# BenjSta/bernoulli-var-speech-codec

Measured on AMD Instinct MI355X. Metric: audio-seconds coded per wall-second (encode+decode), 22.05 kHz @ 3 kbit/s, higher is better.
Workload: dtype f32; 1 GPU; BASELINE configs[1]: batch 64 x 5 s utterances per GPU, config_varBitRate @ 3000 bit/s (35 bits/frame), full encode -> BigVGAN decode; one batch at a time on one stream; frames_per_utterance=430, weights=seeded synthetic (checkpoints are LFS pointers), gather=none, streams=1

## Files before the change

### bernoulli-var-speech-codec_amd/csrc/k_vocoder.hip

```cpp
#include "k_vocoder.h"

namespace bvc {

struct ConvArgs {
    const float *in;  long long Lin;
    float *out;       long long Lout;
    long long in_bs, out_bs;
    long long row_begin;
    const float *res; const float *acc;
    const float *wp;  const float *bias;
    const float *act_a; const float *act_ib;
    float divisor;
    int epi, ks, dil, cout, ntiles, tiles_per_batch;
    const long long *row_lim;
};

template <int CIN, int NTW, int MT, bool NSPLIT = false, int SHIFT = 0>
__global__ __launch_bounds__(256) void conv_mfma_kernel(ConvArgs a) {
    extern __shared__ __attribute__((aligned(16))) float tile[];
    constexpr int S = CIN + 2;
    constexpr int TT = (NSPLIT ? 1 : 4) * MT * 16;
    constexpr int C4 = CIN / 4;
    const int tid = threadIdx.x, lane = tid & 63;
    const int wave = __builtin_amdgcn_readfirstlane(tid >> 6);
    const int r = lane & 15, g = lane >> 4;
    const int b = blockIdx.x / a.tiles_per_batch;
    const long long t0 = a.row_begin + (long long)(blockIdx.x % a.tiles_per_batch) * TT;
    const int ntile0 = NSPLIT ? (blockIdx.y * 4 + wave) * NTW : blockIdx.y * NTW;
    const int halo = (a.ks - 1) * a.dil;
    const int rows = TT + halo;
    const long long lin = a.row_lim ? a.row_lim[b] : a.Lin;

    const float *inb = a.in + (long long)b * a.in_bs;
    for (int idx = tid; idx < rows * C4; idx += 256) {
        const int row = idx / C4, c4 = idx - row * C4;
        const long long tg = t0 - halo + SHIFT + row;
        f32x4 v = (f32x4){0.f, 0.f, 0.f, 0.f};
        if (tg >= 0 && tg < lin) {
            v = *reinterpret_cast<const f32x4 *>(inb + tg * CIN + c4 * 4);
            if (a.act_a) {
                const f32x4 aa = *reinterpret_cast<const f32x4 *>(a.act_a + c4 * 4);
                const f32x4 bb = *reinterpret_cast<const f32x4 *>(a.act_ib + c4 * 4);
#pragma unroll
                for (int e = 0; e < 4; e += 2) {
                    const f32x2 o2 = snakebeta2((f32x2){v[e], v[e + 1]}, (f32x2){aa[e], aa[e + 1]}, (f32x2){bb[e], bb[e + 1]});
                    v[e] = o2[0]; v[e + 1] = o2[1];
                }
            }
        }
        park16<S>(tile, row, c4 * 4, v);
    }
    __syncthreads();

    f32x4 acc[MT][NTW];
#pragma unroll
    for (int i = 0; i < MT; ++i)
#pragma unroll
        for (int n = 0; n < NTW; ++n) acc[i][n] = (f32x4){0.f, 0.f, 0.f, 0.f};

    const int mbase = NSPLIT ? 0 : wave * MT * 16;
    const float *wl = a.wp + (long long)ntile0 * 64 + lane;
    const long long kstride = (long long)a.ntiles * 64;
    bool nok[NTW];
#pragma unroll
    for (int n = 0; n < NTW; ++n) nok[n] = (ntile0 + n) < a.ntiles;

    for (int j = 0; j < a.ks; ++j) {
        const float *arow = tile + (mbase + r + j * a.dil) * S + g;
        const float *wj = wl + (long long)j * C4 * kstride;
        constexpr int CGU = (C4 % 8 == 0) ? 8 : (C4 % 5 == 0) ? 5 : (C4 % 4 == 0) ? 4 : (C4 % 2 == 0) ? 2 : 1;
#pragma unroll 1
        for (int cg0 = 0; cg0 < C4; cg0 += CGU) {
            float bw[CGU][NTW];
#pragma unroll
            for (int u = 0; u < CGU; ++u)
#pragma unroll
                for (int n = 0; n < NTW; ++n)
                    bw[u][n] = nok[n] ? wj[(long long)(cg0 + u) * kstride + n * 64] : 0.0f;
#pragma unroll
            for (int u = 0; u < CGU; ++u) {
                float av[MT];
#pragma unroll
                for (int i = 0; i < MT; ++i) av[i] = arow[i * 16 * S + (cg0 + u) * 4];
#pragma unroll
                for (int i = 0; i < MT; ++i)
#pragma unroll
                    for (int n = 0; n < NTW; ++n)
                        acc[i][n] = __builtin_amdgcn_mfma_f32_16x16x4f32(bw[u][n], av[i], acc[i][n], 0, 0, 0);
            }
        }
    }

    const long long ob = (long long)b * a.out_bs;
#pragma unroll
    for (int i = 0; i < MT; ++i) {
        const long long t = t0 + mbase + i * 16 + r;
        if (t >= a.Lout) continue;
#pragma unroll
        for (int n = 0; n < NTW; ++n) {
            const int col = (ntile0 + n) * 16 + g * 4;
            if (col >= a.cout) continue;
            const long long o = ob + t * a.cout + col;
            f32x4 v = acc[i][n] + *reinterpret_cast<const f32x4 *>(a.bias + col);
            if (a.epi >= CE_RES) v = v + *reinterpret_cast<const f32x4 *>(a.res + o);
            if (a.epi >= CE_RES_ACC) v = *reinterpret_cast<const f32x4 *>(a.acc + o) + v;
            divide_if(a.epi == CE_RES_ACC_DIV, v, a.divisor);
            *reinterpret_cast<f32x4 *>(a.out + o) = v;
        }
    }
}

template <int CIN, int NTW, int MT, bool NSPLIT = false, int SHIFT = 0>
static int launch_one(const ConvArgs &a, int B, hipStream_t s) {
    constexpr int TT = (NSPLIT ? 1 : 4) * MT * 16;
    ConvArgs k = a;
    k.tiles_per_batch = (int)((a.Lout - a.row_begin + TT - 1) / TT);
    if (k.tiles_per_batch <= 0) return BVC_OK;
    const size_t lds = (size_t)(TT + (a.ks - 1) * a.dil) * (CIN + 2) * sizeof(float);
    if (lds > 160 * 1024) { set_error("conv tile needs %zu B of LDS", lds); return BVC_EINVAL; }
    constexpr int NPW = NTW * (NSPLIT ? 4 : 1);
    dim3 grid((unsigned)(k.tiles_per_batch * (long long)B), (unsigned)((a.ntiles + NPW - 1) / NPW));
    auto kern = conv_mfma_kernel<CIN, NTW, MT, NSPLIT, SHIFT>;
    ProbeScope probe(PK_CONV, s);
    hipLaunchKernelGGL(kern, grid, dim3(256), lds, s, k);
    BVC_HIP_TRY(hipGetLastError());
    return BVC_OK;
}

template <int CIN, int NTW, int MT, bool NSPLIT = false, int SHIFT = 0>
static int allow_big_lds() {
    BVC_HIP_TRY(hipFuncSetAttribute(reinterpret_cast<const void *>(conv_mfma_kernel<CIN, NTW, MT, NSPLIT, SHIFT>),
                                    hipFuncAttributeMaxDynamicSharedMemorySize, 160 * 1024));
    return BVC_OK;
}

__global__ void snakebeta_test_kernel(const float *__restrict__ x, long long n, float a, float ib, float *__restrict__ y) {
    for (long long i = ((long long)blockIdx.x * blockDim.x + threadIdx.x) * 2; i < n; i += (long long)gridDim.x * blockDim.x * 2) {
        if (i + 1 < n && !(i & 2)) {
            const f32x2 v = snakebeta2((f32x2){x[i], x[i + 1]}, splat2(a), splat2(ib));
            y[i] = v[0];
            y[i + 1] = v[1];
        } else {
            y[i] = snakebeta(x[i], a, ib);
            if (i + 1 < n) y[i + 1] = snakebeta(x[i + 1], a, ib);
        }
    }
}

int launch_snakebeta_test(const float *x, long long n, float a, float ib, float *y, hipStream_t s) {
    if (n <= 0) return BVC_OK;
    hipLaunchKernelGGL(snakebeta_test_kernel, dim3(256), dim3(256), 0, s, x, n, a, ib, y);
    BVC_HIP_TRY(hipGetLastError());
    return BVC_OK;
}

int conv_kernels_init() {
    int rc;
    if ((rc = amp_kernels_init())) return rc;
    if ((rc = allow_big_lds<512, 4, 1>())) return rc;
    if ((rc = allow_big_lds<512, 4, 1, true>())) return rc;
    if ((rc = allow_big_lds<256, 4, 2>())) return rc;
    if ((rc = allow_big_lds<256, 4, 1, true>())) return rc;
    if ((rc = allow_big_lds<128, 4, 2>())) return rc;
    if ((rc = allow_big_lds<80, 4, 2>())) return rc;
    if ((rc = allow_big_lds<80, 4, 2, false, 3>())) return rc;
    if ((rc = allow_big_lds<64, 4, 2>())) return rc;
    if ((rc = allow_big_lds<32, 2, 4>())) return rc;
    if ((rc = allow_big_lds<16, 1, 4>())) return rc;
    if ((rc = allow_big_lds<8, 1, 4>())) return rc;
    return BVC_OK;
}

int launch_conv_mfma(const ConvLayer &c, const float *in, long long Lin, float *out, long long Lout, int B,
                     int epi, const float *res, const float *acc, float divisor, hipStream_t s, const ConvWindow *win,
                     const long long *row_lim, long long in_bs, int shift) {
    if (B <= 0 || Lout <= 0) return BVC_OK;
    if (c.cout % 4) { set_error("conv_mfma: %d output columns (the epilogue stores 16-byte granules)", c.cout); return BVC_EINVAL; }
    ConvArgs a;
    a.in = in; a.Lin = Lin; a.out = out; a.Lout = Lout; a.res = res; a.acc = acc;
    a.in_bs = win ? win->in_bs : (in_bs ? in_bs : Lin * c.cin);
    a.out_bs = win ? win->out_bs : Lout * c.cout;
    a.row_begin = win ? win->row_begin : 0;
    a.wp = c.wp; a.bias = c.bias; a.act_a = c.act_a; a.act_ib = c.act_ib;
    a.divisor = divisor; a.epi = epi; a.ks = c.ks; a.dil = c.dil; a.cout = c.cout; a.ntiles = c.ntiles;
    a.tiles_per_batch = 0;
    a.row_lim = row_lim;
    if (shift) {
        if (shift != 3 || c.cin != 80 || c.ks != 7 || c.dil != 1 || win || row_lim) { set_error("conv_mfma: a shifted window is conv_pre's (80 channels, 7 taps, shift 3)"); return BVC_EINVAL; }
        return launch_one<80, 4, 2, false, 3>(a, B, s);
    }
    if (win && Lout - a.row_begin <= 16) {
        switch (c.cin) {
            case 512: return launch_one<512, 4, 1, true>(a, B, s);
            case 256: return launch_one<256, 4, 1, true>(a, B, s);
            case 128: return launch_one<128, 4, 1, true>(a, B, s);
            case 80:  return launch_one<80, 2, 1, true>(a, B, s);
            case 64:  return launch_one<64, 4, 1, true>(a, B, s);
            default: break;
        }
    }
    switch (c.cin) {
        case 512: return launch_one<512, 4, 1>(a, B, s);
        case 256: return launch_one<256, 4, 2>(a, B, s);
        case 128: return launch_one<128, 4, 2>(a, B, s);
        case 80:  return launch_one<80, 4, 2>(a, B, s);
        case 64:  return launch_one<64, 4, 2>(a, B, s);
        case 32:  return launch_one<32, 2, 4>(a, B, s);
        case 16:  return launch_one<16, 1, 4>(a, B, s);
        case 8:   return launch_one<8, 1, 4>(a, B, s);
        default:
            set_error("conv_mfma: unsupported input channel count %d", c.cin);
            return BVC_EINVAL;
    }
}

template <int C, int SHIFT = 0>
__global__ __launch_bounds__(256) void conv_post_kernel(const float *__restrict__ in, long long Lin, int ks,
                                                        const float *__restrict__ w, const float *__restrict__ bias,
                                                        const float *__restrict__ act_a,
                                                        const float *__restrict__ act_ib, float div,
                                                        float *__restrict__ wav, long long n_out,
                                                        int tiles_per_batch, long long in_bs, long long row_begin,
                                                        const long long *__restrict__ n_rows) {
    extern __shared__ __attribute__((aligned(16))) float tile[];
    const int tid = threadIdx.x;
    const int b = blockIdx.x / tiles_per_batch;
    const long long t0 = row_begin + (long long)(blockIdx.x % tiles_per_batch) * 256;
    const int halo = ks - 1;
    const float *inb = in + (long long)b * in_bs;
    for (int idx = tid; idx < (256 + halo) * C; idx += 256) {
        const int row = idx / C, c = idx - row * C;
        const long long tg = t0 - halo + SHIFT + row;
        float v = 0.0f;
        if (tg >= 0 && tg < Lin) v = snakebeta(inb[tg * C + c], act_a[c], act_ib[c]);
        tile[idx] = v;
    }
    __syncthreads();
    const long long t = t0 + tid - row_begin;
    if (t >= n_out) return;
    if (n_rows && t >= n_rows[b]) { wav[(long long)b * n_out + t] = 0.0f; return; }
    float acc = 0.0f;
    for (int j = 0; j < ks; ++j)
#pragma unroll
        for (int c = 0; c < C; ++c) acc = fmaf(w[c * ks + j], tile[(tid + j) * C + c], acc);
    wav[(long long)b * n_out + t] = tanhf(acc + bias[0]) / div;
}

template <int C>
__global__ __launch_bounds__(256) void conv_post_aa_kernel(const float *__restrict__ in, long long Lin, int ks,
                                                           const float *__restrict__ w, const float *__restrict__ bias,
                                                           const float *__restrict__ act_a, const float *__restrict__ act_ib,
                                                           const float *__restrict__ fu, const float *__restrict__ fd, float div,
                                                           float *__restrict__ wav, long long n_out, int tiles_per_batch) {
    extern __shared__ __attribute__((aligned(16))) float tile[];
    const int tid = threadIdx.x;
    const int b = blockIdx.x / tiles_per_batch;
    const long long t0 = (long long)(blockIdx.x % tiles_per_batch) * 256;
    const int halo = ks - 1, nact = 256 + halo, nraw = nact + 10;
    float *raw = tile + nact * C;
    const float *inb = in + (long long)b * Lin * C;
    const int first = (int)(t0 - halo) - 5;
    for (int idx = tid; idx < nraw * C; idx += 256) {
        const long long tg = first + idx / C;
        raw[idx] = (tg >= 0 && tg < Lin) ? inb[tg * C + (idx % C)] : 0.0f;
    }
    __syncthreads();
    aa_rows<C>(raw, first, nraw, Lin, tile, first + 5, nact, C, act_a, act_ib, fu, fd);
    __syncthreads();
    const long long t = t0 + tid;
    if (t >= n_out) return;
    float acc = 0.0f;
    for (int j = 0; j < ks; ++j)
#pragma unroll
        for (int c = 0; c < C; ++c) acc = fmaf(w[c * ks + j], tile[(tid + j) * C + c], acc);
    wav[(long long)b * n_out + t] = tanhf(acc + bias[0]) / div;
}

int launch_conv_post(const float *in, long long Lin, int C, int ks, const float *w, const float *bias,
                     const float *act_a, const float *act_ib, float div, float *wav, long long n_out, int B,
                     hipStream_t s, const ConvWindow *win, const long long *n_rows, const float *aa_up, const float *aa_down,
                     bool sym, long long in_bs) {
    if (B <= 0 || n_out <= 0) return BVC_OK;
    if (C != 8 && C != 16 && C != 32) { set_error("conv_post: unsupported channel count %d", C); return BVC_EINVAL; }
    const int tiles = (int)((n_out + 255) / 256);
    if (aa_up || aa_down) {
        if (sym || in_bs) { set_error("conv_post: an anti-aliased activation_post stands in front of a causal conv_post, on a dense signal"); return BVC_EINVAL; }
        if (!aa_up || !aa_down || win || n_rows) { set_error("conv_post: an anti-aliased activation_post has no streaming window and no mixed lengths"); return BVC_EINVAL; }
        if (Lin + 512 > 0x7FFFFFFFll) { set_error("conv_post: %lld rows are beyond the anti-aliased kernel's row index", Lin); return BVC_EINVAL; }
        const size_t lds_aa = (size_t)(2 * (256 + ks - 1) + 10) * C * sizeof(float);
        ProbeScope probe(PK_POST, s);
        auto kern = C == 8 ? conv_post_aa_kernel<8> : C == 16 ? conv_post_aa_kernel<16> : conv_post_aa_kernel<32>;
        if (C == 32) {
            static bool attr = false;
            if (!attr) { BVC_HIP_TRY(hipFuncSetAttribute(reinterpret_cast<const void *>(conv_post_aa_kernel<32>), hipFuncAttributeMaxDynamicSharedMemorySize, 160 * 1024)); attr = true; }
        }
        hipLaunchKernelGGL(kern, dim3((unsigned)(tiles * (long long)B)), dim3(256), lds_aa, s, in, Lin, ks,
                           w, bias, act_a, act_ib, aa_up, aa_down, div, wav, n_out, tiles);
        BVC_HIP_TRY(hipGetLastError());
        return BVC_OK;
    }
    const size_t lds = (size_t)(256 + ks - 1) * C * sizeof(float);
    if (sym && (win || n_rows || ks != 7)) { set_error("conv_post: a symmetric conv_post has 7 taps, no streaming window and no mixed lengths"); return BVC_EINVAL; }
    ProbeScope probe(PK_POST, s);
    auto kern = sym ? (C == 8 ? conv_post_kernel<8, 3> : C == 16 ? conv_post_kernel<16, 3> : conv_post_kernel<32, 3>)
                    : (C == 8 ? conv_post_kernel<8> : C == 16 ? conv_post_kernel<16> : conv_post_kernel<32>);
    hipLaunchKernelGGL(kern, dim3((unsigned)(tiles * (long long)B)), dim3(256), lds, s, in, Lin, ks,
                       w, bias, act_a, act_ib, div, wav, n_out, tiles, win ? win->in_bs : (in_bs ? in_bs : Lin * C), win ? win->row_begin : 0, n_rows);
    BVC_HIP_TRY(hipGetLastError());
    return BVC_OK;
}

struct UpRates { int u[8]; };
__global__ void ragged_limits_kernel(long long *__restrict__ lim, const long long *__restrict__ frames,
                                     const long long *__restrict__ lengths, int B, long long T, long long n_max, int n_up, UpRates r) {
    const int b = blockIdx.x * blockDim.x + threadIdx.x;
    if (b >= B) return;
    const long long f = frames[b] < 0 ? 0 : (frames[b] > T ? T : frames[b]);
    long long L = f;
    for (int i = 0; i < n_up; ++i) {
        lim[(long long)i * B + b] = L;
        L = (L + 1) * r.u[i];
    }
    long long n = lengths[b] < L ? lengths[b] : L;
    n = f == 0 ? 0 : (n < 0 ? 0 : (n > n_max ? n_max : n));
    lim[(long long)n_up * B + b] = n;
}

int launch_ragged_limits(long long *lim, const long long *frames, const long long *lengths, int B, long long T, long long n_max,
                         int n_up, const int *up_rates, hipStream_t s) {
    if (B <= 0) return BVC_OK;
    if (n_up > 8) { set_error("ragged limits: %d upsamplers", n_up); return BVC_EINVAL; }
    UpRates r;
    for (int i = 0; i < 8; ++i) r.u[i] = i < n_up ? up_rates[i] : 0;
    hipLaunchKernelGGL(ragged_limits_kernel, dim3((B + 255) / 256), dim3(256), 0, s, lim, frames, lengths, B, T, n_max, n_up, r);
    BVC_HIP_TRY(hipGetLastError());
    return BVC_OK;
}
}
```

Before: 7088 audio-seconds/s.

## Reuse staged input tile across column groups in MFMA conv and post kernel

Adds a conv_rows kernel that stages the activated input row tile in LDS once and then loops over several output column groups per block, so input loads and snake activations are no longer repeated for every column block. It also prefetches weight fragments one step ahead, swizzles block order across groups of eight, and loads input through bounds-checked buffer loads in batches of 16-byte vectors. The non-MFMA conv_post kernel gets the same vectorized buffer loading and stores its tile channel-major with padding to reduce LDS bank conflicts. The trade-offs are fewer blocks in the grid, with less parallelism for narrow layers, and more register pressure from the double-buffered weights.

After: 7100 audio-seconds/s (median of 6 runs). Within noise of the previous version (+0.2%).

```diff
diff --git a/bernoulli-var-speech-codec_amd/csrc/k_vocoder.hip b/bernoulli-var-speech-codec_amd/csrc/k_vocoder.hip
--- a/bernoulli-var-speech-codec_amd/csrc/k_vocoder.hip
+++ b/bernoulli-var-speech-codec_amd/csrc/k_vocoder.hip
@@ -13,7 +13,20 @@
     float divisor;
     int epi, ks, dil, cout, ntiles, tiles_per_batch;
     const long long *row_lim;
+    unsigned nrt;
+    int ncg;
 };
+
+struct SpanRows { __amdgpu_buffer_rsrc_t rs; int row0; };
+__device__ __forceinline__ SpanRows span_rows(const float *item, long long lin, long long first, int rows, int C) {
+    const long long in0 = first > 0 ? first : 0;
+    long long n = (first + rows < lin ? first + rows : lin) - in0;
+    if (n < 0) n = 0;
+    return {__builtin_amdgcn_make_buffer_rsrc(const_cast<float *>(item + in0 * C), 0, (int)(n * C * 4), 0x00020000), (int)(in0 - first)};
+}
+__device__ __forceinline__ f32x4 span_load4(const SpanRows &sp, int row, int C, int c0) {
+    return __builtin_bit_cast(f32x4, __builtin_amdgcn_raw_buffer_load_b128(sp.rs, ((row - sp.row0) * C + c0) * 4, 0, 0));
+}
 
 template <int CIN, int NTW, int MT, bool NSPLIT = false, int SHIFT = 0>
 __global__ __launch_bounds__(256) void conv_mfma_kernel(ConvArgs a) {
@@ -110,6 +123,166 @@
     }
 }
 
+constexpr int conv_rows_waves(int CIN) { return CIN <= 32 ? 4 : 1; }
+template <int CIN, int NTW, int MT, int SHIFT = 0>
+__global__ __launch_bounds__(256, conv_rows_waves(CIN)) void conv_rows_kernel(ConvArgs a) {
+    extern __shared__ __attribute__((aligned(16))) float tile[];
+    constexpr int S = CIN + 2;
+    constexpr int TT = 4 * MT * 16;
+    constexpr int C4 = CIN / 4;
+    constexpr int CGU = (C4 % 8 == 0) ? 8 : (C4 % 5 == 0) ? 5 : (C4 % 4 == 0) ? 4 : (C4 % 2 == 0) ? 2 : 1;
+    constexpr int CPT = C4 / CGU;
+    const int tid = threadIdx.x, lane = tid & 63;
+    const int wave = __builtin_amdgcn_readfirstlane(tid >> 6);
+    const int r = lane & 15, g = lane >> 4;
+    const unsigned per = gridDim.x >> 3;
+    const unsigned bid = (blockIdx.x & 7u) * per + (blockIdx.x >> 3);
+    if (bid >= a.nrt) return;
+    const int b = (int)(bid / (unsigned)a.tiles_per_batch);
+    const long long t0 = a.row_begin + (long long)(bid - (unsigned)b * (unsigned)a.tiles_per_batch) * TT;
+    const int halo = (a.ks - 1) * a.dil;
+    const int rows = TT + halo;
+    const long long lin = a.row_lim ? a.row_lim[b] : a.Lin;
+
+    const int cg_first = blockIdx.y * a.ncg;
+    const int ncgs = (a.ntiles + NTW - 1) / NTW;
+    const int cg_end = cg_first + a.ncg < ncgs ? cg_first + a.ncg : ncgs;
+    const int nch = a.ks * CPT;
+    const float *wl = a.wp + lane;
+    float bcur[CGU][NTW], bnxt[CGU][NTW];
+    auto loadb = [&](float (&dstb)[CGU][NTW], int cg, int q) {
+#pragma unroll
+        for (int n = 0; n < NTW; ++n) {
+            const int nt = cg * NTW + n < a.ntiles ? cg * NTW + n : a.ntiles - 1;
+#pragma unroll
+            for (int u = 0; u < CGU; ++u) dstb[u][n] = wl[((q * CGU + u) * a.ntiles + nt) * 64];
+        }
+    };
+    loadb(bcur, cg_first, 0);
+
+    {
+        constexpr int NLD0 = ((TT + 1) * C4 + 255) / 256;
+        constexpr int NTRIP = (NLD0 + 11) / 12, NB = (NLD0 + NTRIP - 1) / NTRIP;
+        const SpanRows sp = span_rows(a.in + (long long)b * a.in_bs, lin, t0 - halo + SHIFT, rows, CIN);
+        const int total = rows * C4;
+#pragma unroll 1
+        for (int base = tid; base < total; base += 256 * NB) {
+            f32x4 v[NB];
+#pragma unroll
+            for (int i = 0; i < NB; ++i) {
+                const int idx = base + i * 256;
+                const int row = idx / C4, c4 = idx - row * C4;
+                v[i] = span_load4(sp, row, CIN, c4 * 4);
+            }
+#pragma unroll
+            for (int i = 0; i < NB; ++i) {
+                const int idx = base + i * 256;
+                if (idx < total) {
+                    const int row = idx / C4, c4 = idx - row * C4;
+                    f32x4 o = v[i];
+                    if (a.act_a) {
+                        const f32x4 aa = *reinterpret_cast<const f32x4 *>(a.act_a + c4 * 4);
+                        const f32x4 bb = *reinterpret_cast<const f32x4 *>(a.act_ib + c4 * 4);
+#pragma unroll
+                        for (int e = 0; e < 4; e += 2) {
+                            const f32x2 o2 = snakebeta2((f32x2){o[e], o[e + 1]}, (f32x2){aa[e], aa[e + 1]}, (f32x2){bb[e], bb[e + 1]});
+                            o[e] = o2[0]; o[e + 1] = o2[1];
+                        }
+                    }
+                    park16<S>(tile, row, c4 * 4, o);
+                }
+            }
+        }
+    }
+    __syncthreads();
+
+    const int mbase = wave * MT * 16;
+    const long long ob = (long long)b * a.out_bs;
+#pragma unroll 1
+    for (int cg = cg_first; cg < cg_end; ++cg) {
+        f32x4 acc[MT][NTW];
+#pragma unroll
+        for (int i = 0; i < MT; ++i)
+#pragma unroll
+            for (int n = 0; n < NTW; ++n) acc[i][n] = (f32x4){0.f, 0.f, 0.f, 0.f};
+        f32x4 bv[NTW];
+#pragma unroll
+        for (int n = 0; n < NTW; ++n) {
+            const int col = (cg * NTW + n) * 16 + g * 4;
+            bv[n] = *reinterpret_cast<const f32x4 *>(a.bias + (col < a.cout ? col : a.cout - 4));
+        }
+#pragma unroll 1
+        for (int q = 0; q < nch; ++q) {
+            const bool last = q + 1 == nch;
+            loadb(bnxt, last ? (cg + 1 < cg_end ? cg + 1 : cg) : cg, last ? 0 : q + 1);
+            __builtin_amdgcn_sched_barrier(0);
+            const int j = q / CPT, cg0 = (q - j * CPT) * CGU;
+            const float *arow = tile + (mbase + r + j * a.dil) * S + g + cg0 * 4;
+#pragma unroll
+            for (int u = 0; u < CGU; ++u) {
+                float av[MT];
+#pragma unroll
+                for (int i = 0; i < MT; ++i) av[i] = arow[i * 16 * S + u * 4];
+#pragma unroll
+                for (int i = 0; i < MT; ++i)
+#pragma unroll
+                    for (int n = 0; n < NTW; ++n)
+                        acc[i][n] = __builtin_amdgcn_mfma_f32_16x16x4f32(bcur[u][n], av[i], acc[i][n], 0, 0, 0);
+            }
+            __builtin_amdgcn_sched_barrier(0);
+#pragma unroll
+            for (int u = 0; u < CGU; ++u)
+#pragma unroll
+                for (int n = 0; n < NTW; ++n) bcur[u][n] = bnxt[u][n];
+        }
+
+#pragma unroll
+        for (int i = 0; i < MT; ++i) {
+            const long long t = t0 + mbase + i * 16 + r;
+            if (t >= a.Lout) continue;
+#pragma unroll
+            for (int n = 0; n < NTW; ++n) {
+                const int col = (cg * NTW + n) * 16 + g * 4;
+                if (col >= a.cout) continue;
+                const long long o = ob + t * a.cout + col;
+                f32x4 v = acc[i][n] + bv[n];
+                if (a.epi >= CE_RES) v = v + *reinterpret_cast<const f32x4 *>(a.res + o);
+                if (a.epi >= CE_RES_ACC) v = *reinterpret_cast<const f32x4 *>(a.acc + o) + v;
+                divide_if(a.epi == CE_RES_ACC_DIV, v, a.divisor);
+                *reinterpret_cast<f32x4 *>(a.out + o) = v;
+            }
+        }
+    }
+}
+
+constexpr int CONV_NCG = 4;
+
+template <int CIN, int NTW, int MT, int SHIFT = 0>
+static int launch_rows(const ConvArgs &a, int B, hipStream_t s) {
+    constexpr int TT = 4 * MT * 16;
+    ConvArgs k = a;
+    const long long tpb = (a.Lout - a.row_begin + TT - 1) / TT;
+    if (tpb <= 0) return BVC_OK;
+    if (tpb * B > 0x7FFFFFF0ll) { set_error("conv: %lld row tiles", tpb * B); return BVC_EINVAL; }
+    k.tiles_per_batch = (int)tpb;
+    k.nrt = (unsigned)(tpb * B);
+    const size_t lds = (size_t)(TT + (a.ks - 1) * a.dil) * (CIN + 2) * sizeof(float);
+    if (lds > 160 * 1024) { set_error("conv tile needs %zu B of LDS", lds); return BVC_EINVAL; }
+    const int ncgs = (a.ntiles + NTW - 1) / NTW;
+    k.ncg = ncgs <= 2 ? 1 : (ncgs < CONV_NCG ? ncgs : CONV_NCG);
+    dim3 grid((k.nrt + 7u) & ~7u, (unsigned)((ncgs + k.ncg - 1) / k.ncg));
+    ProbeScope probe(PK_CONV, s);
+    hipLaunchKernelGGL((conv_rows_kernel<CIN, NTW, MT, SHIFT>), grid, dim3(256), lds, s, k);
+    BVC_HIP_TRY(hipGetLastError());
+    return BVC_OK;
+}
+template <int CIN, int NTW, int MT, int SHIFT = 0>
+static int allow_big_lds_rows() {
+    BVC_HIP_TRY(hipFuncSetAttribute(reinterpret_cast<const void *>(conv_rows_kernel<CIN, NTW, MT, SHIFT>),
+                                    hipFuncAttributeMaxDynamicSharedMemorySize, 160 * 1024));
+    return BVC_OK;
+}
+
 template <int CIN, int NTW, int MT, bool NSPLIT = false, int SHIFT = 0>
 static int launch_one(const ConvArgs &a, int B, hipStream_t s) {
     constexpr int TT = (NSPLIT ? 1 : 4) * MT * 16;
@@ -157,17 +330,17 @@
 int conv_kernels_init() {
     int rc;
     if ((rc = amp_kernels_init())) return rc;
-    if ((rc = allow_big_lds<512, 4, 1>())) return rc;
     if ((rc = allow_big_lds<512, 4, 1, true>())) return rc;
-    if ((rc = allow_big_lds<256, 4, 2>())) return rc;
     if ((rc = allow_big_lds<256, 4, 1, true>())) return rc;
-    if ((rc = allow_big_lds<128, 4, 2>())) return rc;
-    if ((rc = allow_big_lds<80, 4, 2>())) return rc;
-    if ((rc = allow_big_lds<80, 4, 2, false, 3>())) return rc;
-    if ((rc = allow_big_lds<64, 4, 2>())) return rc;
-    if ((rc = allow_big_lds<32, 2, 4>())) return rc;
-    if ((rc = allow_big_lds<16, 1, 4>())) return rc;
-    if ((rc = allow_big_lds<8, 1, 4>())) return rc;
+    if ((rc = allow_big_lds_rows<512, 4, 1>())) return rc;
+    if ((rc = allow_big_lds_rows<256, 4, 2>())) return rc;
+    if ((rc = allow_big_lds_rows<128, 4, 2>())) return rc;
+    if ((rc = allow_big_lds_rows<80, 4, 2>())) return rc;
+    if ((rc = allow_big_lds_rows<80, 4, 2, 3>())) return rc;
+    if ((rc = allow_big_lds_rows<64, 4, 2>())) return rc;
+    if ((rc = allow_big_lds_rows<32, 2, 4>())) return rc;
+    if ((rc = allow_big_lds_rows<16, 1, 4>())) return rc;
+    if ((rc = allow_big_lds_rows<8, 1, 4>())) return rc;
     return BVC_OK;
 }
 
@@ -187,7 +360,7 @@
     a.row_lim = row_lim;
     if (shift) {
         if (shift != 3 || c.cin != 80 || c.ks != 7 || c.dil != 1 || win || row_lim) { set_error("conv_mfma: a shifted window is conv_pre's (80 channels, 7 taps, shift 3)"); return BVC_EINVAL; }
-        return launch_one<80, 4, 2, false, 3>(a, B, s);
+        return launch_rows<80, 4, 2, 3>(a, B, s);
     }
     if (win && Lout - a.row_begin <= 16) {
         switch (c.cin) {
@@ -200,19 +373,21 @@
         }
     }
     switch (c.cin) {
-        case 512: return launch_one<512, 4, 1>(a, B, s);
-        case 256: return launch_one<256, 4, 2>(a, B, s);
-        case 128: return launch_one<128, 4, 2>(a, B, s);
-        case 80:  return launch_one<80, 4, 2>(a, B, s);
-        case 64:  return launch_one<64, 4, 2>(a, B, s);
-        case 32:  return launch_one<32, 2, 4>(a, B, s);
-        case 16:  return launch_one<16, 1, 4>(a, B, s);
-        case 8:   return launch_one<8, 1, 4>(a, B, s);
+        case 512: return launch_rows<512, 4, 1>(a, B, s);
+        case 256: return launch_rows<256, 4, 2>(a, B, s);
+        case 128: return launch_rows<128, 4, 2>(a, B, s);
+        case 80:  return launch_rows<80, 4, 2>(a, B, s);
+        case 64:  return launch_rows<64, 4, 2>(a, B, s);
+        case 32:  return launch_rows<32, 2, 4>(a, B, s);
+        case 16:  return launch_rows<16, 1, 4>(a, B, s);
+        case 8:   return launch_rows<8, 1, 4>(a, B, s);
         default:
             set_error("conv_mfma: unsupported input channel count %d", c.cin);
             return BVC_EINVAL;
     }
 }
+
+__host__ __device__ static inline int post_plane(int C, int ks) { return ((256 + ks - 1 + 7) & ~7) + 32 / C; }
 
 template <int C, int SHIFT = 0>
 __global__ __launch_bounds__(256) void conv_post_kernel(const float *__restrict__ in, long long Lin, int ks,
@@ -223,17 +398,35 @@
                                                         int tiles_per_batch, long long in_bs, long long row_begin,
                                                         const long long *__restrict__ n_rows) {
     extern __shared__ __attribute__((aligned(16))) float tile[];
+    constexpr int C4 = C / 4;
     const int tid = threadIdx.x;
     const int b = blockIdx.x / tiles_per_batch;
     const long long t0 = row_begin + (long long)(blockIdx.x % tiles_per_batch) * 256;
     const int halo = ks - 1;
-    const float *inb = in + (long long)b * in_bs;
-    for (int idx = tid; idx < (256 + halo) * C; idx += 256) {
-        const int row = idx / C, c = idx - row * C;
-        const long long tg = t0 - halo + SHIFT + row;
-        float v = 0.0f;
-        if (tg >= 0 && tg < Lin) v = snakebeta(inb[tg * C + c], act_a[c], act_ib[c]);
-        tile[idx] = v;
+    const int rows = 256 + halo, total = rows * C4;
+    const int P = post_plane(C, ks);
+    const SpanRows sp = span_rows(in + (long long)b * in_bs, Lin, t0 - halo + SHIFT, rows, C);
+    constexpr int NB = (262 * C4 + 255) / 256;
+#pragma unroll 1
+    for (int base = tid; base < total; base += 256 * NB) {
+        f32x4 v[NB];
+#pragma unroll
+        for (int i = 0; i < NB; ++i) {
+            const int idx = base + i * 256;
+            const int row = idx / C4, c4 = idx - row * C4;
+            v[i] = span_load4(sp, row, C, c4 * 4);
+        }
+#pragma unroll
+        for (int i = 0; i < NB; ++i) {
+            const int idx = base + i * 256;
+            if (idx < total) {
+                const int row = idx / C4, c4 = idx - row * C4;
+                const f32x4 aa = *reinterpret_cast<const f32x4 *>(act_a + c4 * 4);
+                const f32x4 bb = *reinterpret_cast<const f32x4 *>(act_ib + c4 * 4);
+#pragma unroll
+                for (int e = 0; e < 4; ++e) tile[(c4 * 4 + e) * P + row] = snakebeta(v[i][e], aa[e], bb[e]);
+            }
+        }
     }
     __syncthreads();
     const long long t = t0 + tid - row_begin;
@@ -242,7 +435,7 @@
     float acc = 0.0f;
     for (int j = 0; j < ks; ++j)
 #pragma unroll
-        for (int c = 0; c < C; ++c) acc = fmaf(w[c * ks + j], tile[(tid + j) * C + c], acc);
+        for (int c = 0; c < C; ++c) acc = fmaf(w[c * ks + j], tile[c * P + tid + j], acc);
     wav[(long long)b * n_out + t] = tanhf(acc + bias[0]) / div;
 }
 
@@ -299,7 +492,7 @@
         BVC_HIP_TRY(hipGetLastError());
         return BVC_OK;
     }
-    const size_t lds = (size_t)(256 + ks - 1) * C * sizeof(float);
+    const size_t lds = (size_t)post_plane(C, ks) * C * sizeof(float);
     if (sym && (win || n_rows || ks != 7)) { set_error("conv_post: a symmetric conv_post has 7 taps, no streaming window and no mixed lengths"); return BVC_EINVAL; }
     ProbeScope probe(PK_POST, s);
     auto kern = sym ? (C == 8 ? conv_post_kernel<8, 3> : C == 16 ? conv_post_kernel<16, 3> : conv_post_kernel<32, 3>)
```
